# retrojetpacks/Gadget-Leicester

Measured on AMD Instinct MI355X. Metric: particle-steps/sec (gravity+SPH), higher is better.
Workload: dtype f64

## Files before the change

gadget-leicester_amd/csrc/ghip_walk.h:

```cpp
#pragma once
#include "ghip_internal.h"
#include "ghip_count.h"

#ifndef GHIP_WALK_WAVES
#define GHIP_WALK_WAVES 8
#endif
#ifndef GHIP_WALK_OPT
#define GHIP_WALK_OPT 15
#endif


struct GravK
{
  double theta;
  double errtol;
  double boxsize, boxhalf;
  int periodic, unequal;
  int debug_steps;
  int xcd_remap;
  double rcut, rcut2, asmthfac;
  double fac_intp;
  double k1875;
};

__device__ int *d_walk_errw = nullptr;

#include "ghip_walkrec.h"

typedef double v16i __attribute__((ext_vector_type(8)));

struct __attribute__((aligned(8))) EwPair
{
  double lo, hi;
};
__device__ __forceinline__ EwPair d_ldpair(const double *p)
{
  return *reinterpret_cast<const EwPair *>(p);
}

__device__ __forceinline__ double d_f64(const v16i &v, int i)
{
  return v[i];
}
__device__ __forceinline__ int d_lo32(const v16i &v, int i)
{
  return __double2loint(v[i]);
}
__device__ __forceinline__ int d_hi32(const v16i &v, int i)
{
  return __double2hiint(v[i]);
}

__device__ __forceinline__ unsigned int d_rec_off(int e)
{
  return (unsigned int) __builtin_amdgcn_readfirstlane(e) << 6;
}
template <class T>
__device__ __forceinline__ void d_load1(const T *__restrict__ base, int e, v16i &R)
{
  const unsigned int off = d_rec_off(e);
  asm volatile("s_load_dwordx16 %0, %1, %2\n\ts_waitcnt lgkmcnt(0)" : "=s"(R) : "s"(base), "s"(off) : "memory");
}
template <class T>
__device__ __forceinline__ void d_load2(const T *__restrict__ base, int ea, v16i &A, int eb, v16i &B)
{
  const unsigned int oa = d_rec_off(ea), ob = d_rec_off(eb);
  asm volatile("s_load_dwordx16 %0, %2, %3\n\ts_load_dwordx16 %1, %2, %4\n\ts_waitcnt lgkmcnt(0)"
               : "=&s"(A), "=&s"(B)
               : "s"(base), "s"(oa), "s"(ob)
               : "memory");
}
template <class T>
__device__ __forceinline__ void d_touch_next(const T *__restrict__ base, unsigned int off, int &scratch)
{
  asm volatile("s_load_dword %0, %1, %2 offset:0x40" : "=s"(scratch) : "s"(base), "s"(off) : "memory");
}
template <class T>
__device__ __forceinline__ void d_touch(const T *__restrict__ base, int e, int &scratch)
{
  const unsigned int off = d_rec_off(e);
  asm volatile("s_load_dword %0, %1, %2" : "=s"(scratch) : "s"(base), "s"(off) : "memory");
}
template <class T>
__device__ __forceinline__ void d_load1_touch(const T *__restrict__ base, unsigned int off, v16i &R,
                                              int &s1, int &s2)
{
  asm volatile("s_load_dwordx16 %0, %3, %4\n\ts_waitcnt lgkmcnt(0)"
               : "=s"(R), "+s"(s1), "+s"(s2)
               : "s"(base), "s"(off)
               : "memory");
}
__device__ __forceinline__ void d_drain_touch(int &s1, int &s2)
{
  asm volatile("s_waitcnt lgkmcnt(0) ; drain-touches" : "+s"(s1), "+s"(s2) : : "memory");
}

__device__ __forceinline__ double d_rsqrt(double x)
{
  double y = __builtin_amdgcn_rsq(x);
  double t = x * y;
  double e = fma(-t, y, 1.0);
  double p = fma(0.375, e, 0.5);
  return fma(y * e, p, y);
}

__device__ __forceinline__ double d_mass_over_r3(double mass, double x, double k15 = 1.5,
                                                 double k1875 = 1.875)
{
  double y = __builtin_amdgcn_rsq(x);
  double y2 = y * y;
  double e = fma(-x, y2, 1.0);
  double p = fma(k1875, e, k15);
  double c = (mass * y) * y2;
  return fma(c * e, p, c);
}

__device__ __forceinline__ double d_grav_fac(double mass, double r2, double h, double h2,
                                             double &r_out)
{
  if(r2 >= h2)
    {
      double rinv = d_rsqrt(r2);
      r_out = r2 * rinv;
      return mass * rinv * rinv * rinv;
    }
  double r = sqrt(r2);
  r_out = r;
  double h_inv = 1.0 / h;
  double h3_inv = h_inv * h_inv * h_inv;
  double u = r * h_inv;
  if(u < 0.5)
    return mass * h3_inv * (10.666666666667 + u * u * (32.0 * u - 38.4));
  return mass * h3_inv *
         (21.333333333333 - 48.0 * u + 38.4 * u * u - 10.666666666667 * u * u * u -
          0.066666666667 / (u * u * u));
}

template <bool BRICK>
__device__ __forceinline__ void d_ewald_interp(const double *__restrict__ tab, double fac_intp,
                                               double dx, double dy, double dz, double &fx,
                                               double &fy, double &fz)
{
  const int E1 = GHIP_EN + 1;
  const double sx = dx < 0 ? 1.0 : -1.0, sy = dy < 0 ? 1.0 : -1.0, sz = dz < 0 ? 1.0 : -1.0;
  dx = fabs(dx);
  dy = fabs(dy);
  dz = fabs(dz);
  double u = dx * fac_intp;
  int i = (int) u;
  if(i >= GHIP_EN)
    i = GHIP_EN - 1;
  u -= i;
  double v = dy * fac_intp;
  int j = (int) v;
  if(j >= GHIP_EN)
    j = GHIP_EN - 1;
  v -= j;
  double w = dz * fac_intp;
  int k = (int) w;
  if(k >= GHIP_EN)
    k = GHIP_EN - 1;
  w -= k;
  double f1 = (1 - u) * (1 - v) * (1 - w), f2 = (1 - u) * (1 - v) * (w);
  double f3 = (1 - u) * (v) * (1 - w), f4 = (1 - u) * (v) * (w);
  double f5 = (u) * (1 - v) * (1 - w), f6 = (u) * (1 - v) * (w);
  double f7 = (u) * (v) * (1 - w), f8 = (u) * (v) * (w);
  EwPair x00, x01, x10, x11, y00, y01, y10, y11, z00, z01, z10, z11;
  if(!BRICK)
    {
      const unsigned int ui = (unsigned int) i, uj = (unsigned int) j, uk = (unsigned int) k;
      const unsigned int R1 = E1 * 8u, R2 = E1 * E1 * 8u;
      const unsigned int ox = (ui * E1 + uj) * R1 + uk * 8u;
      const unsigned int oy = (uj * E1 + ui) * R1 + uk * 8u;
      const unsigned int oz = (uk * E1 + uj) * R1 + ui * 8u;
      const unsigned int ox2 = ox + R2, oy2 = oy + R2, oz2 = oz + R2;
      const char *tb = reinterpret_cast<const char *>(tab);
#define EW_LD(off, imm) d_ldpair(reinterpret_cast<const double *>(tb + (size_t) (off) + (imm)))
      x00 = EW_LD(ox, 0), x01 = EW_LD(ox, R1), x10 = EW_LD(ox2, 0), x11 = EW_LD(ox2, R1);
      y00 = EW_LD(oy, 0), y01 = EW_LD(oy, R1), y10 = EW_LD(oy2, 0), y11 = EW_LD(oy2, R1);
      z00 = EW_LD(oz, 0), z01 = EW_LD(oz, R1), z10 = EW_LD(oz2, 0), z11 = EW_LD(oz2, R1);
#undef EW_LD
    }
  else
    {
      const unsigned int SA = GHIP_EW_NB * GHIP_EW_NKB * 128, SB = GHIP_EW_NKB * 128;
      const unsigned int ai = (i >> 1) * SA + (i & 1) * 64, ai1 = ((i + 1) >> 1) * SA + ((i + 1) & 1) * 64;
      const unsigned int aj = (j >> 1) * SA + (j & 1) * 64, aj1 = ((j + 1) >> 1) * SA + ((j + 1) & 1) * 64;
      const unsigned int ak = (k >> 1) * SA + (k & 1) * 64, ak1 = ((k + 1) >> 1) * SA + ((k + 1) & 1) * 64;
      const unsigned int bi = (i >> 1) * SB + (i & 1) * 32, bi1 = ((i + 1) >> 1) * SB + ((i + 1) & 1) * 32;
      const unsigned int bj = (j >> 1) * SB + (j & 1) * 32, bj1 = ((j + 1) >> 1) * SB + ((j + 1) & 1) * 32;
      const unsigned int ck = ((((unsigned int) k * 43u) >> 7) * 13u + (unsigned int) k) * 8u;
      const unsigned int ci = ((((unsigned int) i * 43u) >> 7) * 13u + (unsigned int) i) * 8u;
      const char *tb = reinterpret_cast<const char *>(tab);
#define EW_LD(off) d_ldpair(reinterpret_cast<const double *>(tb + (off)))
      x00 = EW_LD(ai + bj + ck), x01 = EW_LD(ai + bj1 + ck), x10 = EW_LD(ai1 + bj + ck),
      x11 = EW_LD(ai1 + bj1 + ck);
      y00 = EW_LD(aj + bi + ck), y01 = EW_LD(aj + bi1 + ck), y10 = EW_LD(aj1 + bi + ck),
      y11 = EW_LD(aj1 + bi1 + ck);
      z00 = EW_LD(ak + bj + ci), z01 = EW_LD(ak + bj1 + ci), z10 = EW_LD(ak1 + bj + ci),
      z11 = EW_LD(ak1 + bj1 + ci);
#undef EW_LD
    }
  fx = sx * (x00.lo * f1 + x00.hi * f2 + x01.lo * f3 + x01.hi * f4 + x10.lo * f5 + x10.hi * f6 +
             x11.lo * f7 + x11.hi * f8);
  fy = sy * (y00.lo * f1 + y00.hi * f2 + y10.lo * f3 + y10.hi * f4 + y01.lo * f5 + y01.hi * f6 +
             y11.lo * f7 + y11.hi * f8);
  fz = sz * (z00.lo * f1 + z10.lo * f2 + z01.lo * f3 + z11.lo * f4 + z00.hi * f5 + z10.hi * f6 +
             z01.hi * f7 + z11.hi * f8);
}

struct WalkLane
{
  double pos_x, pos_y, pos_z, h_i, aold;
  double h2;
  double k15;
  double acc_x, acc_y, acc_z;
  int nint;
};

__device__ __forceinline__ double d_nearest1(double x, double boxsize, double boxhalf)
{
  return (fabs(x) > boxhalf) ? x - copysign(boxsize, x) : x;
}

__device__ __forceinline__ double d_nearest1_masked(double x, double boxsize, double boxhalf)
{
  if(fabs(x) > boxhalf)
    {
      x -= copysign(boxsize, x);
      asm volatile("" : "+v"(x));
    }
  return x;
}

typedef unsigned long long lmask;
#define D_BAL(cond) __builtin_amdgcn_ballot_w64(cond)
#define D_LANE(mask) __builtin_amdgcn_inverse_ballot_w64(mask)

__device__ __forceinline__ void d_skip_to(int &my_skip, int skip)
{
  asm volatile("v_max_i32 %0, %1, %0" : "+v"(my_skip) : "s"(skip));
}

template <int MODE, bool PERIODIC, bool UNEQUAL, bool OWNED, bool REL>
__device__ __forceinline__ int d_walk_element(int e, const v16i &H,
                                              const WalkCold *__restrict__ cold, const GravK &p,
                                              const float *__restrict__ srtab,
                                              const double *__restrict__ ewtab, WalkLane &W,
                                              int &my_skip)
{
  const double ex = d_f64(H, 0), ey = d_f64(H, 1), ez = d_f64(H, 2), mass = d_f64(H, 3);
  const double mlen2 = d_f64(H, 4), len2 = d_f64(H, 5);
  const int skip = d_lo32(H, 6), pidx = d_hi32(H, 6);
  const double aux = d_f64(H, 7);
  const lmask act = D_BAL(e >= my_skip);
  int next;

  double dx = ex - W.pos_x, dy = ey - W.pos_y, dz = ez - W.pos_z;
  double r2;
  if((GHIP_WALK_OPT & 1) && (MODE == GHIP_WALK_EWALD || PERIODIC))
    {
      r2 = dx * dx + dy * dy + dz * dz;
      if(D_BAL(r2 >= p.boxhalf * p.boxhalf) != 0)
        {
          if(D_LANE(D_BAL(fabs(dx) > p.boxhalf)))
            {
              dx -= copysign(p.boxsize, dx);
              asm volatile("" : "+v"(dx));
            }
          if(D_LANE(D_BAL(fabs(dy) > p.boxhalf)))
            {
              dy -= copysign(p.boxsize, dy);
              asm volatile("" : "+v"(dy));
            }
          if(D_LANE(D_BAL(fabs(dz) > p.boxhalf)))
            {
              dz -= copysign(p.boxsize, dz);
              asm volatile("" : "+v"(dz));
            }
          r2 = dx * dx + dy * dy + dz * dz;
        }
    }
  else if(MODE == GHIP_WALK_EWALD || PERIODIC)
    {
      const lmask wx = D_BAL(fabs(dx) > p.boxhalf), wy = D_BAL(fabs(dy) > p.boxhalf),
                  wz = D_BAL(fabs(dz) > p.boxhalf);
      if((wx | wy | wz) != 0)
        {
          if(D_LANE(wx))
            {
              dx -= copysign(p.boxsize, dx);
              asm volatile("" : "+v"(dx));
            }
          if(D_LANE(wy))
            {
              dy -= copysign(p.boxsize, dy);
              asm volatile("" : "+v"(dy));
            }
          if(D_LANE(wz))
            {
              dz -= copysign(p.boxsize, dz);
              asm volatile("" : "+v"(dz));
            }
        }
      r2 = dx * dx + dy * dy + dz * dz;
    }
  else
    r2 = dx * dx + dy * dy + dz * dz;
  double h = W.h_i, h2 = W.h2;
  lmask interact;

  if(pidx >= 0)
    {
      next = e + 1;
      interact = act;
      if(MODE != GHIP_WALK_EWALD && UNEQUAL)
        {
          if(h < aux)
            {
              h = aux;
              h2 = h * h;
            }
        }
    }
  else
    {
      lmask gt, rel;
      if(REL)
        {
          gt = D_BAL(mlen2 > r2 * r2 * W.aold);
          rel = ~0ull;
        }
      else
        {
          gt = D_BAL(len2 > r2 * p.theta * p.theta);
          rel = 0ull;
        }
      lmask open = act & gt;
      lmask far = act & ~gt & rel;
      lmask drop = 0;
      const double len2x4 = __hiloint2double(d_hi32(H, 5) + 0x00200000, d_lo32(H, 5));
      const lmask boxcand = far & D_BAL(r2 < len2x4);
      lmask cutcand = 0;
      if(MODE == GHIP_WALK_SHORTRANGE)
        cutcand = act & D_BAL(r2 > p.rcut2);
      lmask need_cold = boxcand;
      if(MODE == GHIP_WALK_SHORTRANGE)
        need_cold |= cutcand;
      if(MODE == GHIP_WALK_EWALD)
        need_cold |= open;
      if(need_cold != 0)
        {
          v16i C;
          d_load1(cold, e, C);
          const double cx = d_f64(C, 0), cy = d_f64(C, 1), cz = d_f64(C, 2), len = d_f64(C, 3);
          const double len06 = d_f64(C, 4);
          const double c0 = cx - W.pos_x, c1 = cy - W.pos_y, c2 = cz - W.pos_z;
          if(MODE == GHIP_WALK_SHORTRANGE)
            {
              if(cutcand != 0)
                {
                  double eff = p.rcut + 0.5 * len;
                  double d0 = c0, d1 = c1, d2 = c2;
                  if(PERIODIC)
                    {
                      d0 = d_nearest1(d0, p.boxsize, p.boxhalf);
                      d1 = d_nearest1(d1, p.boxsize, p.boxhalf);
                      d2 = d_nearest1(d2, p.boxsize, p.boxhalf);
                    }
                  drop = cutcand &
                         (D_BAL(fabs(d0) > eff) | D_BAL(fabs(d1) > eff) | D_BAL(fabs(d2) > eff));
                }
              open &= ~drop;
              far &= ~drop;
            }
          if(far != 0)
            open |= far & D_BAL(fabs(c0) < len06) & D_BAL(fabs(c1) < len06) &
                    D_BAL(fabs(c2) < len06);
          if(MODE == GHIP_WALK_EWALD)
            {
              if(open != 0 && !(len > 0.20 * p.boxsize))
                {
                  double u0 = d_nearest1(c0, p.boxsize, p.boxhalf);
                  double u1 = d_nearest1(c1, p.boxsize, p.boxhalf);
                  double u2 = d_nearest1(c2, p.boxsize, p.boxhalf);
                  double lim = 0.5 * (p.boxsize - len);
                  open &= D_BAL(fabs(u0) > lim) | D_BAL(fabs(u1) > lim) | D_BAL(fabs(u2) > lim);
                }
            }
        }
      if(MODE != GHIP_WALK_EWALD && UNEQUAL)
        {
          const double ms = fabs(aux);
          const lmask up = act & ~drop & ~open & D_BAL(h < ms);
          if(up != 0)
            {
              if(D_LANE(up))
                {
                  h = ms;
                  h2 = ms * ms;
                }
              if(aux < 0)
                open |= up & D_BAL(r2 < ms * ms);
            }
        }
      interact = act & ~drop & ~open;
      if(!((GHIP_WALK_OPT & 4) && OWNED && MODE == GHIP_WALK_NEWTON) || (interact & D_BAL(r2 < h2)) != 0)
        if(D_LANE(interact | drop))
          d_skip_to(my_skip, skip);
      next = skip;
      if(open != 0)
        {
          next = e + 1;
          if(skip == next)
            {
              int *w = *(int *volatile *) &d_walk_errw;
              if(w)
                *(volatile int *) w = 1;
            }
        }
    }

  if(OWNED && MODE == GHIP_WALK_NEWTON && (interact & D_BAL(r2 < h2)) == 0)
    {
      const int counted = pidx & 1;
      const int sk = skip;
      if(D_LANE(interact))
        {
          const double fac = (GHIP_WALK_OPT & 8) ? d_mass_over_r3(mass, r2, W.k15, p.k1875)
                                                 : d_mass_over_r3(mass, r2);
          W.acc_x += dx * fac;
          W.acc_y += dy * fac;
          W.acc_z += dz * fac;
          if(GHIP_WALK_OPT & 2)
            W.nint += counted;
          else
            W.nint += (mass > 0) ? 1 : 0;
          if(GHIP_WALK_OPT & 4)
            d_skip_to(my_skip, sk);
        }
      return next;
    }
  if(OWNED && D_LANE(interact))
    {
      if(MODE == GHIP_WALK_EWALD)
        {
          double fx, fy, fz;
          d_ewald_interp<UNEQUAL>(ewtab, p.fac_intp, dx, dy, dz, fx, fy, fz);
          W.acc_x += mass * fx;
          W.acc_y += mass * fy;
          W.acc_z += mass * fz;
          W.nint++;
        }
      else
        {
          double r;
          double fac = d_grav_fac(mass, r2, h, h2, r);
          if(MODE == GHIP_WALK_SHORTRANGE)
            {
              int tabindex = (int) (p.asmthfac * r);
              if(tabindex < GHIP_NTAB)
                {
                  fac *= srtab[tabindex];
                  W.acc_x += dx * fac;
                  W.acc_y += dy * fac;
                  W.acc_z += dz * fac;
                  W.nint++;
                }
            }
          else
            {
              W.acc_x += dx * fac;
              W.acc_y += dy * fac;
              W.acc_z += dz * fac;
              if(mass > 0)
                W.nint++;
            }
        }
    }
  return next;
}

struct WalkPlan
{
  int nwaves;
  const int *__restrict__ wave_bucket;
  const int *__restrict__ woff;
  const int *__restrict__ nsub;
  unsigned int *__restrict__ steps_out;
  unsigned int *started;
  int started_at;
};

struct SegCursor
{
  int kseg;
  int e, s1;
};

template <int MODE, bool PERIODIC, bool UNEQUAL, bool REL>
__device__ __forceinline__ bool d_enter_segment(SegCursor &c, int stride, const WalkSeg &sg,
                                                const WalkHot *__restrict__ hot,
                                                const WalkCold *__restrict__ cold, const GravK &p,
                                                const float *__restrict__ srtab,
                                                const double *__restrict__ ewtab, bool valid,
                                                WalkLane &W, int &my_skip, unsigned int &steps)
{
  while(c.kseg < sg.ns)
    {
      const int s0 = __builtin_amdgcn_readfirstlane(sg.start[c.kseg]);
      c.s1 = __builtin_amdgcn_readfirstlane(sg.start[c.kseg + 1]);
      my_skip = valid ? 0 : 0x7fffffff;
      const int na = __builtin_amdgcn_readfirstlane(sg.nanc[c.kseg]);
      for(int a = 0; a < na; a++)
        {
          int ea = __builtin_amdgcn_readfirstlane(sg.anc[c.kseg * GHIP_MAXANC + a]);
          v16i H;
          d_load1(hot, ea, H);
          d_walk_element<MODE, PERIODIC, UNEQUAL, false, REL>(ea, H, cold, p, srtab, ewtab, W, my_skip);
          steps++;
        }
      int first = d_wave_min_i32(my_skip);
      c.e = __builtin_amdgcn_readfirstlane(first > s0 ? first : s0);
      if(c.e < c.s1)
        return true;
      c.kseg += stride;
    }
  return false;
}

template <int MODE, bool PERIODIC, bool UNEQUAL, bool REL>
__device__ __forceinline__ void d_walk_run(const WalkSeg &sg, int sub, const WalkHot *__restrict__ hot,
                                           const WalkCold *__restrict__ cold, const GravK &p,
                                           const float *__restrict__ srtab,
                                           const double *__restrict__ ewtab, bool valid, WalkLane &W,
                                           unsigned int &steps)
{
  if(MODE != GHIP_WALK_EWALD)
    {
      SegCursor A;
      int skipA = 0;
      A.kseg = sub;
      const int stride = sg.nsub;
      bool liveA = d_enter_segment<MODE, PERIODIC, UNEQUAL, REL>(A, stride, sg, hot, cold, p, srtab,
                                                            ewtab, valid, W, skipA, steps);
      int t1 = 0, t2 = 0;
      while(liveA)
        {
          v16i HA;
          const unsigned int offA = d_rec_off(A.e);
          d_load1_touch(hot, offA, HA, t1, t2);
          d_touch_next(hot, offA, t1);
          d_touch(hot, d_lo32(HA, 6), t2);
          steps++;
          A.e = __builtin_amdgcn_readfirstlane(
            d_walk_element<MODE, PERIODIC, UNEQUAL, true, REL>(A.e, HA, cold, p, srtab, ewtab, W, skipA));
          if(A.e >= A.s1)
            {
              d_drain_touch(t1, t2);
              A.kseg += stride;
              liveA = d_enter_segment<MODE, PERIODIC, UNEQUAL, REL>(A, stride, sg, hot, cold, p, srtab,
                                                               ewtab, valid, W, skipA, steps);
            }
        }
      d_drain_touch(t1, t2);
    }
  else
    {
      SegCursor A, B;
      int skipA = 0, skipB = 0;
      A.kseg = sub;
      B.kseg = sub + sg.nsub;
      const int stride = 2 * sg.nsub;
      bool liveA = d_enter_segment<MODE, PERIODIC, UNEQUAL, REL>(A, stride, sg, hot, cold, p, srtab, ewtab, valid,
                                                   W, skipA, steps);
      bool liveB = d_enter_segment<MODE, PERIODIC, UNEQUAL, REL>(B, stride, sg, hot, cold, p, srtab, ewtab, valid,
                                                   W, skipB, steps);
      while(liveA && liveB)
        {
          v16i HA, HB;
          d_load2(hot, A.e, HA, B.e, HB);
          steps += 2;
          A.e = __builtin_amdgcn_readfirstlane(
            d_walk_element<MODE, PERIODIC, UNEQUAL, true, REL>(A.e, HA, cold, p, srtab, ewtab, W, skipA));
          B.e = __builtin_amdgcn_readfirstlane(
            d_walk_element<MODE, PERIODIC, UNEQUAL, true, REL>(B.e, HB, cold, p, srtab, ewtab, W, skipB));
          if(A.e >= A.s1)
            {
              A.kseg += stride;
              liveA = d_enter_segment<MODE, PERIODIC, UNEQUAL, REL>(A, stride, sg, hot, cold, p, srtab, ewtab,
                                                      valid, W, skipA, steps);
            }
          if(B.e >= B.s1)
            {
              B.kseg += stride;
              liveB = d_enter_segment<MODE, PERIODIC, UNEQUAL, REL>(B, stride, sg, hot, cold, p, srtab, ewtab,
                                                      valid, W, skipB, steps);
            }
        }
      if(liveB)
        {
          A = B;
          skipA = skipB;
          liveA = true;
        }
      while(liveA)
        {
          v16i HA;
          d_load1(hot, A.e, HA);
          steps++;
          A.e = __builtin_amdgcn_readfirstlane(
            d_walk_element<MODE, PERIODIC, UNEQUAL, true, REL>(A.e, HA, cold, p, srtab, ewtab, W, skipA));
          if(A.e >= A.s1)
            {
              A.kseg += stride;
              liveA = d_enter_segment<MODE, PERIODIC, UNEQUAL, REL>(A, stride, sg, hot, cold, p, srtab, ewtab,
                                                      valid, W, skipA, steps);
            }
        }
    }

}

template <int MODE, bool PERIODIC, bool UNEQUAL>
__global__ void __launch_bounds__(GHIP_BLOCK) __attribute__((amdgpu_waves_per_eu(MODE == GHIP_WALK_EWALD ? 4 : GHIP_WALK_WAVES, 8)))
k_grav_walk(int nelem, const WalkHot *__restrict__ hot, const WalkCold *__restrict__ cold,
            WalkSeg sg, int nt, const int *__restrict__ tgt, const double *__restrict__ tx,
            const double *__restrict__ ty, const double *__restrict__ tz,
            const double *__restrict__ tsoft, const double *__restrict__ toldacc, GravK p,
            const float *__restrict__ srtab, const double *__restrict__ ewtab,
            double *__restrict__ pax, double *__restrict__ pay, double *__restrict__ paz,
            int *__restrict__ pcost, unsigned long long *__restrict__ counter,
            unsigned long long *__restrict__ acc, WalkPlan plan)
{
  const int lane = threadIdx.x & 63;
  if(plan.started && blockIdx.x == plan.started_at && threadIdx.x == 0)
    __hip_atomic_store(plan.started, 1u, __ATOMIC_RELEASE, __HIP_MEMORY_SCOPE_SYSTEM);
  const int per_xcd = gridDim.x >> 3;
  int lblock = blockIdx.x;
  if(p.xcd_remap == 1)
    lblock = (blockIdx.x & 7) * per_xcd + (blockIdx.x >> 3);
  else if(p.xcd_remap > 1)
    {
      const int j = blockIdx.x >> 3, x = blockIdx.x & 7, G = p.xcd_remap;
      lblock = ((j / G) * 8 + x) * G + (j % G);
    }
  const int wave = __builtin_amdgcn_readfirstlane((lblock * (int) blockDim.x + threadIdx.x) >> 6);
  if(wave >= plan.nwaves)
    return;
  const int bucket = __builtin_amdgcn_readfirstlane(plan.wave_bucket[wave]);
  if(bucket < 0 || bucket * 64 >= nt)
    return;
  const int sub = wave - __builtin_amdgcn_readfirstlane(plan.woff[bucket]);
  sg.nsub = __builtin_amdgcn_readfirstlane(plan.nsub[bucket]);
  const int ti = bucket * 64 + lane;
  const bool valid = ti < nt;
  const int s = valid ? (tgt ? tgt[ti] : ti) : 0;

  WalkLane W;
  W.pos_x = W.pos_y = W.pos_z = 0;
  W.h_i = 1;
  W.aold = 0;
  W.h2 = 1;
  if(valid)
    {
      W.pos_x = tx[s];
      W.pos_y = ty[s];
      W.pos_z = tz[s];
      W.h_i = tsoft[s];
      W.aold = p.errtol * toldacc[s];
      W.h2 = W.h_i * W.h_i;
    }
  W.acc_x = W.acc_y = W.acc_z = 0;
  W.nint = 0;
  W.k15 = 1.5;
  asm volatile("" : "+v"(W.k15));
  unsigned int steps = 0;

  if(p.theta == 0)
    d_walk_run<MODE, PERIODIC, UNEQUAL, true>(sg, sub, hot, cold, p, srtab, ewtab, valid, W, steps);
  else
    d_walk_run<MODE, PERIODIC, UNEQUAL, false>(sg, sub, hot, cold, p, srtab, ewtab, valid, W, steps);

  if(valid)
    {
      const size_t o = (size_t) wave * 64 + lane;
      pax[o] = W.acc_x;
      pay[o] = W.acc_y;
      paz[o] = W.acc_z;
      pcost[o] = p.debug_steps ? (int) steps : W.nint;
    }
  unsigned long long tot = d_wave_sum_u64((unsigned long long) W.nint);
  if(lane == 0 && tot && counter)
    {
      d_count(counter, 0, tot);
      d_count(acc, 0, tot);
    }
  if(lane == 0)
    {
      if(counter)
        {
          d_count(counter, 1, (unsigned long long) steps);
          d_count(acc, 1, (unsigned long long) steps);
        }
      atomicAdd(plan.steps_out + bucket, steps);
    }
}

__global__ void k_plan_nsub(int nb, int ns, int sbase, const unsigned int *__restrict__ steps_prev,
                            int nprev, int *__restrict__ nsub)
{
  __shared__ unsigned long long part[4];
  unsigned long long tot = 0;
  if(nprev > 0)
    {
      for(int k = threadIdx.x; k < nprev; k += blockDim.x)
        tot += steps_prev[k];
      for(int o = 32; o > 0; o >>= 1)
        tot += __shfl_xor(tot, o);
      if((threadIdx.x & 63) == 0)
        part[threadIdx.x >> 6] = tot;
      __syncthreads();
      tot = part[0] + part[1] + part[2] + part[3];
    }
  int b = blockIdx.x * blockDim.x + threadIdx.x;
  if(b >= nb)
    return;
  int s = ns < sbase ? ns : sbase;
  if(b < nprev && tot > 0)
    {
      double mean = (double) tot / (double) nprev;
      s = (int) ((double) sbase * (double) steps_prev[b] / mean) + 1;
      s = s < 2 ? 2 : s;
      s = s > 64 ? 64 : s;
      if(s > ns)
        s = ns;
    }
  nsub[b] = s < 1 ? 1 : s;
}

__global__ void k_plan_fill(int nb, const int *__restrict__ nsub, const int *__restrict__ woff,
                            int maxwaves, int *__restrict__ wave_bucket,
                            unsigned int *__restrict__ steps_out, int *__restrict__ errword)
{
  int b = blockIdx.x * blockDim.x + threadIdx.x;
  if(b >= nb)
    return;
  int o = woff[b], s = nsub[b];
  if(o + s > maxwaves)
    *(volatile int *) errword = 1;
  for(int q = 0; q < s; q++)
    if(o + q < maxwaves)
      wave_bucket[o + q] = b;
  steps_out[b] = 0;
}

struct SegTables
{
  int ntab;
  int ns[3], soff[3], noff[3];
};

__global__ void k_build_segments(const TreeSizes *__restrict__ ts, const int4 *__restrict__ lk,
                                 SegTables T, int *__restrict__ start, int *__restrict__ nanc,
                                 int *__restrict__ anc)
{
  const int nelem = ts->nelem;
  int g = blockIdx.x * blockDim.x + threadIdx.x;
  int j = 0;
  while(j < T.ntab && g > T.ns[j])
    {
      g -= T.ns[j] + 1;
      j++;
    }
  if(j >= T.ntab)
    return;
  const int ns = T.ns[j], k = g;
  start += T.soff[j];
  nanc += T.noff[j];
  anc += (size_t) T.noff[j] * GHIP_MAXANC;
  long long chunk = ((long long) nelem + ns - 1) / ns;
  long long s0l = (long long) k * chunk;
  int s0 = (int) (s0l > nelem ? nelem : s0l);
  if(k == ns)
    s0 = nelem;
  start[k] = s0;
  if(k == ns)
    return;
  int na = 0, e = 0;
  while(e < s0)
    {
      int4 q = lk[e];
      if(!LK_IS_PARTICLE(q) && q.x > s0)
        {
          if(na < GHIP_MAXANC)
            anc[k * GHIP_MAXANC + na] = e;
          na++;
          e = e + 1;
        }
      else
        e = q.x;
    }
  nanc[k] = na < GHIP_MAXANC ? na : GHIP_MAXANC;
}

__global__ void k_combine_grav(int nt, WalkPlan plan, const int *__restrict__ tgt,
                               const int *__restrict__ perm, const double *__restrict__ pax,
                               const double *__restrict__ pay, const double *__restrict__ paz,
                               const int *__restrict__ pcost, int n, double *__restrict__ oacc,
                               int *__restrict__ ocost, int accumulate, int debug_max)
{
  int ti = blockIdx.x * blockDim.x + threadIdx.x;
  if(ti >= nt)
    return;
  const int bucket = ti >> 6, lane = ti & 63;
  const int w0 = plan.woff[bucket];
  int nsub = plan.nsub[bucket];
  if(w0 + nsub > plan.nwaves)
    nsub = plan.nwaves > w0 ? plan.nwaves - w0 : 0;
  double a0 = 0, a1 = 0, a2 = 0;
  int c = 0;
  for(int s = 0; s < nsub; s++)
    {
      size_t o = (size_t) (w0 + s) * 64 + lane;
      a0 += pax[o];
      a1 += pay[o];
      a2 += paz[o];
      c = debug_max ? (pcost[o] > c ? pcost[o] : c) : c + pcost[o];
    }
  int i = perm ? perm[tgt[ti]] : ti;
  if(accumulate)
    {
      oacc[i] += a0;
      oacc[(size_t) n + i] += a1;
      oacc[2 * (size_t) n + i] += a2;
      ocost[i] += c;
    }
  else
    {
      oacc[i] = a0;
      oacc[(size_t) n + i] = a1;
      oacc[2 * (size_t) n + i] = a2;
      ocost[i] = c;
    }
}

__global__ void k_combine_pair(int nt, WalkPlan pn, WalkPlan pe, const int *__restrict__ tgt,
                               const int *__restrict__ perm, const double *__restrict__ nax,
                               const double *__restrict__ nay, const double *__restrict__ naz,
                               const int *__restrict__ ncost, const double *__restrict__ eax,
                               const double *__restrict__ eay, const double *__restrict__ eaz,
                               const int *__restrict__ ecost, int n, double *__restrict__ oacc,
                               int *__restrict__ ocost)
{
  int ti = blockIdx.x * blockDim.x + threadIdx.x;
  if(ti >= nt)
    return;
  const int bucket = ti >> 6, lane = ti & 63;
  double a0 = 0, a1 = 0, a2 = 0, b0 = 0, b1 = 0, b2 = 0;
  int c = 0, d = 0;
  {
    const int w0 = pn.woff[bucket];
    int nsub = pn.nsub[bucket];
    if(w0 + nsub > pn.nwaves)
      nsub = pn.nwaves > w0 ? pn.nwaves - w0 : 0;
    for(int s = 0; s < nsub; s++)
      {
        size_t o = (size_t) (w0 + s) * 64 + lane;
        a0 += nax[o];
        a1 += nay[o];
        a2 += naz[o];
        c += ncost[o];
      }
  }
  {
    const int w0 = pe.woff[bucket];
    int nsub = pe.nsub[bucket];
    if(w0 + nsub > pe.nwaves)
      nsub = pe.nwaves > w0 ? pe.nwaves - w0 : 0;
    for(int s = 0; s < nsub; s++)
      {
        size_t o = (size_t) (w0 + s) * 64 + lane;
        b0 += eax[o];
        b1 += eay[o];
        b2 += eaz[o];
        d += ecost[o];
      }
  }
  int i = perm ? perm[tgt[ti]] : ti;
  oacc[i] = a0 + b0;
  oacc[(size_t) n + i] = a1 + b1;
  oacc[2 * (size_t) n + i] = a2 + b2;
  ocost[i] = c + d;
}

__global__ void k_fill_elems(const TreeSizes *__restrict__ ts, const double4 *__restrict__ xm,
                             const double4 *__restrict__ cl, const int4 *__restrict__ lk,
                             const double *__restrict__ aux, WalkHot *__restrict__ hot,
                             WalkCold *__restrict__ cold)
{
  int e = blockIdx.x * blockDim.x + threadIdx.x;
  if(e >= ts->nelem)
    return;
  double4 v = xm[e], c = cl[e];
  int4 k = lk[e];
  WalkHot h;
  h.x = v.x;
  h.y = v.y;
  h.z = v.z;
  h.m = v.w;
  WalkCold q;
  q.cx = c.x;
  q.cy = c.y;
  q.cz = c.z;
  q.len = c.w;
  if(LK_IS_PARTICLE(k))
    {
      h.mlen2 = 0.0;
      h.len2 = 0.0;
      q.len06 = 0.0;
    }
  else
    {
      h.mlen2 = v.w * c.w * c.w;
      h.len2 = c.w * c.w;
      q.len06 = 0.60 * c.w;
    }
  h.skip = k.x;
  h.pidx = (LK_IS_PARTICLE(k) ? 0 : (int) 0x80000000) | (v.w > 0 ? 1 : 0);
  h.aux = aux[e];
  q.spare[0] = q.spare[1] = q.spare[2] = 0.0;
  hot[e] = h;
  cold[e] = q;
}
```

Baseline: 83.12 million.

## Restructure Ewald table addressing and move skip updates into interaction blocks

Moves the Ewald table address computation into a shared helper that uses 24-bit multiplies and a base offset plus immediate form, so the 12 loads can use constant offsets. In the tree walk, the per-lane skip-pointer update is moved into the force-accumulation branches for Newton and Ewald modes. The softened Newton case gets its own branch instead of falling through to the general path. It also switches to a masked nearest-image helper in the Ewald opening test. The goal is fewer address instructions and less divergent control flow per walk step. The cost is extra branches, and the result relies on the new helpers producing the same addresses as before.

```diff
diff --git a/gadget-leicester_amd/csrc/ghip_ewaddr.h b/gadget-leicester_amd/csrc/ghip_ewaddr.h
--- /dev/null
+++ b/gadget-leicester_amd/csrc/ghip_ewaddr.h
@@ -0,0 +1,54 @@
+#pragma once
+
+#if defined(__HIP_DEVICE_COMPILE__) && __HIP_DEVICE_COMPILE__
+#define GHIP_EW_UMUL(a, b) __umul24((a), (b))
+#define GHIP_EW_IMUL(a, b) __mul24((a), (b))
+#else
+#define GHIP_EW_UMUL(a, b) ((unsigned int) (a) * (unsigned int) (b))
+#define GHIP_EW_IMUL(a, b) ((int) (a) * (int) (b))
+#endif
+#ifdef __HIPCC__
+#define GHIP_EW_FN static inline __host__ __device__ __attribute__((always_inline))
+#else
+#define GHIP_EW_FN static inline
+#endif
+
+GHIP_EW_FN void ghip_ew_brick_addr(int i, int j, int k, unsigned int off[12], unsigned int imm[12])
+{
+  const unsigned int SA = GHIP_EW_NB * GHIP_EW_NKB * 128, SB = GHIP_EW_NKB * 128;
+  const unsigned int ui = (unsigned int) i, uj = (unsigned int) j, uk = (unsigned int) k;
+  const int pi = i & 1, pj = j & 1, pk = k & 1;
+  const unsigned int ai = (unsigned int) (GHIP_EW_IMUL(pi, 64 - (int) (SA / 2)) + (int) GHIP_EW_UMUL(ui, SA / 2));
+  const unsigned int aj = (unsigned int) (GHIP_EW_IMUL(pj, 64 - (int) (SA / 2)) + (int) GHIP_EW_UMUL(uj, SA / 2));
+  const unsigned int ak = (unsigned int) (GHIP_EW_IMUL(pk, 64 - (int) (SA / 2)) + (int) GHIP_EW_UMUL(uk, SA / 2));
+  const unsigned int ai1 = GHIP_EW_UMUL((unsigned int) pi, SA - 128) + ai;
+  const unsigned int aj1 = GHIP_EW_UMUL((unsigned int) pj, SA - 128) + aj;
+  const unsigned int ak1 = GHIP_EW_UMUL((unsigned int) pk, SA - 128) + ak;
+  const unsigned int bi = (unsigned int) (GHIP_EW_IMUL(pi, 32 - (int) (SB / 2)) + (int) GHIP_EW_UMUL(ui, SB / 2));
+  const unsigned int bj = (unsigned int) (GHIP_EW_IMUL(pj, 32 - (int) (SB / 2)) + (int) GHIP_EW_UMUL(uj, SB / 2));
+  const unsigned int bi1 = GHIP_EW_UMUL((unsigned int) pi, SB - 64) + bi;
+  const unsigned int bj1 = GHIP_EW_UMUL((unsigned int) pj, SB - 64) + bj;
+  const unsigned int ck = (GHIP_EW_UMUL(GHIP_EW_UMUL(uk, 43u) >> 7, 13u) + uk) * 8u;
+  const unsigned int ci = (GHIP_EW_UMUL(GHIP_EW_UMUL(ui, 43u) >> 7, 13u) + ui) * 8u;
+  off[0] = ai + bj + ck, off[1] = ai + bj1 + ck, off[2] = ai1 + bj + ck, off[3] = ai1 + bj1 + ck;
+  off[4] = aj + bi + ck, off[5] = aj + bi1 + ck, off[6] = aj1 + bi + ck, off[7] = aj1 + bi1 + ck;
+  off[8] = ak + bj + ci, off[9] = ak + bj1 + ci, off[10] = ak1 + bj + ci, off[11] = ak1 + bj1 + ci;
+  for(int q = 0; q < 12; q++)
+    imm[q] = (q & 1) * 32u + ((q >> 1) & 1) * 64u;
+}
+
+GHIP_EW_FN void ghip_ew_rows_addr(int i, int j, int k, unsigned int off[12], unsigned int imm[12])
+{
+  const unsigned int R1 = (GHIP_EN + 1) * 8u, R2 = (GHIP_EN + 1) * (GHIP_EN + 1) * 8u;
+  const unsigned int ui = (unsigned int) i, uj = (unsigned int) j, uk = (unsigned int) k;
+  const unsigned int E1 = GHIP_EN + 1;
+  const unsigned int ox = GHIP_EW_UMUL(GHIP_EW_UMUL(ui, E1) + uj, R1) + uk * 8u;
+  const unsigned int oy = GHIP_EW_UMUL(GHIP_EW_UMUL(uj, E1) + ui, R1) + uk * 8u;
+  const unsigned int oz = GHIP_EW_UMUL(GHIP_EW_UMUL(uk, E1) + uj, R1) + ui * 8u;
+  for(int q = 0; q < 12; q++)
+    {
+      const unsigned int o = q < 4 ? ox : q < 8 ? oy : oz;
+      off[q] = o + ((q >> 1) & 1) * R2;
+      imm[q] = (q & 1) * R1;
+    }
+}
diff --git a/gadget-leicester_amd/csrc/ghip_walk.h b/gadget-leicester_amd/csrc/ghip_walk.h
--- a/gadget-leicester_amd/csrc/ghip_walk.h
+++ b/gadget-leicester_amd/csrc/ghip_walk.h
@@ -1,6 +1,7 @@
 #pragma once
 #include "ghip_internal.h"
 #include "ghip_count.h"
+#include "ghip_ewaddr.h"
 
 #ifndef GHIP_WALK_WAVES
 #define GHIP_WALK_WAVES 8
@@ -166,41 +167,17 @@
   double f5 = (u) * (1 - v) * (1 - w), f6 = (u) * (1 - v) * (w);
   double f7 = (u) * (v) * (1 - w), f8 = (u) * (v) * (w);
   EwPair x00, x01, x10, x11, y00, y01, y10, y11, z00, z01, z10, z11;
-  if(!BRICK)
-    {
-      const unsigned int ui = (unsigned int) i, uj = (unsigned int) j, uk = (unsigned int) k;
-      const unsigned int R1 = E1 * 8u, R2 = E1 * E1 * 8u;
-      const unsigned int ox = (ui * E1 + uj) * R1 + uk * 8u;
-      const unsigned int oy = (uj * E1 + ui) * R1 + uk * 8u;
-      const unsigned int oz = (uk * E1 + uj) * R1 + ui * 8u;
-      const unsigned int ox2 = ox + R2, oy2 = oy + R2, oz2 = oz + R2;
-      const char *tb = reinterpret_cast<const char *>(tab);
-#define EW_LD(off, imm) d_ldpair(reinterpret_cast<const double *>(tb + (size_t) (off) + (imm)))
-      x00 = EW_LD(ox, 0), x01 = EW_LD(ox, R1), x10 = EW_LD(ox2, 0), x11 = EW_LD(ox2, R1);
-      y00 = EW_LD(oy, 0), y01 = EW_LD(oy, R1), y10 = EW_LD(oy2, 0), y11 = EW_LD(oy2, R1);
-      z00 = EW_LD(oz, 0), z01 = EW_LD(oz, R1), z10 = EW_LD(oz2, 0), z11 = EW_LD(oz2, R1);
+  unsigned int off[12], imm[12];
+  if(BRICK)
+    ghip_ew_brick_addr(i, j, k, off, imm);
+  else
+    ghip_ew_rows_addr(i, j, k, off, imm);
+  const char *tb = reinterpret_cast<const char *>(tab);
+#define EW_LD(q) d_ldpair(reinterpret_cast<const double *>(tb + (size_t) off[q] + imm[q]))
+  x00 = EW_LD(0), x01 = EW_LD(1), x10 = EW_LD(2), x11 = EW_LD(3);
+  y00 = EW_LD(4), y01 = EW_LD(5), y10 = EW_LD(6), y11 = EW_LD(7);
+  z00 = EW_LD(8), z01 = EW_LD(9), z10 = EW_LD(10), z11 = EW_LD(11);
 #undef EW_LD
-    }
-  else
-    {
-      const unsigned int SA = GHIP_EW_NB * GHIP_EW_NKB * 128, SB = GHIP_EW_NKB * 128;
-      const unsigned int ai = (i >> 1) * SA + (i & 1) * 64, ai1 = ((i + 1) >> 1) * SA + ((i + 1) & 1) * 64;
-      const unsigned int aj = (j >> 1) * SA + (j & 1) * 64, aj1 = ((j + 1) >> 1) * SA + ((j + 1) & 1) * 64;
-      const unsigned int ak = (k >> 1) * SA + (k & 1) * 64, ak1 = ((k + 1) >> 1) * SA + ((k + 1) & 1) * 64;
-      const unsigned int bi = (i >> 1) * SB + (i & 1) * 32, bi1 = ((i + 1) >> 1) * SB + ((i + 1) & 1) * 32;
-      const unsigned int bj = (j >> 1) * SB + (j & 1) * 32, bj1 = ((j + 1) >> 1) * SB + ((j + 1) & 1) * 32;
-      const unsigned int ck = ((((unsigned int) k * 43u) >> 7) * 13u + (unsigned int) k) * 8u;
-      const unsigned int ci = ((((unsigned int) i * 43u) >> 7) * 13u + (unsigned int) i) * 8u;
-      const char *tb = reinterpret_cast<const char *>(tab);
-#define EW_LD(off) d_ldpair(reinterpret_cast<const double *>(tb + (off)))
-      x00 = EW_LD(ai + bj + ck), x01 = EW_LD(ai + bj1 + ck), x10 = EW_LD(ai1 + bj + ck),
-      x11 = EW_LD(ai1 + bj1 + ck);
-      y00 = EW_LD(aj + bi + ck), y01 = EW_LD(aj + bi1 + ck), y10 = EW_LD(aj1 + bi + ck),
-      y11 = EW_LD(aj1 + bi1 + ck);
-      z00 = EW_LD(ak + bj + ci), z01 = EW_LD(ak + bj1 + ci), z10 = EW_LD(ak1 + bj + ci),
-      z11 = EW_LD(ak1 + bj1 + ci);
-#undef EW_LD
-    }
   fx = sx * (x00.lo * f1 + x00.hi * f2 + x01.lo * f3 + x01.hi * f4 + x10.lo * f5 + x10.hi * f6 +
              x11.lo * f7 + x11.hi * f8);
   fy = sy * (y00.lo * f1 + y00.hi * f2 + y10.lo * f3 + y10.hi * f4 + y01.lo * f5 + y01.hi * f6 +
@@ -309,6 +286,7 @@
     r2 = dx * dx + dy * dy + dz * dz;
   double h = W.h_i, h2 = W.h2;
   lmask interact;
+  lmask took = 0;
 
   if(pidx >= 0)
     {
@@ -381,9 +359,9 @@
             {
               if(open != 0 && !(len > 0.20 * p.boxsize))
                 {
-                  double u0 = d_nearest1(c0, p.boxsize, p.boxhalf);
-                  double u1 = d_nearest1(c1, p.boxsize, p.boxhalf);
-                  double u2 = d_nearest1(c2, p.boxsize, p.boxhalf);
+                  double u0 = d_nearest1_masked(c0, p.boxsize, p.boxhalf);
+                  double u1 = d_nearest1_masked(c1, p.boxsize, p.boxhalf);
+                  double u2 = d_nearest1_masked(c2, p.boxsize, p.boxhalf);
                   double lim = 0.5 * (p.boxsize - len);
                   open &= D_BAL(fabs(u0) > lim) | D_BAL(fabs(u1) > lim) | D_BAL(fabs(u2) > lim);
                 }
@@ -405,9 +383,7 @@
             }
         }
       interact = act & ~drop & ~open;
-      if(!((GHIP_WALK_OPT & 4) && OWNED && MODE == GHIP_WALK_NEWTON) || (interact & D_BAL(r2 < h2)) != 0)
-        if(D_LANE(interact | drop))
-          d_skip_to(my_skip, skip);
+      took = interact | drop;
       next = skip;
       if(open != 0)
         {
@@ -421,11 +397,34 @@
         }
     }
 
-  if(OWNED && MODE == GHIP_WALK_NEWTON && (interact & D_BAL(r2 < h2)) == 0)
-    {
+  const bool skip_in_block =
+    OWNED && ((MODE == GHIP_WALK_NEWTON && (GHIP_WALK_OPT & 4)) || MODE == GHIP_WALK_EWALD);
+  if(!skip_in_block)
+    if(D_LANE(took))
+      d_skip_to(my_skip, skip);
+
+  if(OWNED && MODE == GHIP_WALK_NEWTON)
+    {
+      lmask plain = interact;
+      if((interact & D_BAL(r2 < h2)) != 0)
+        {
+          if(D_LANE(interact))
+            {
+              double r;
+              const double fac = d_grav_fac(mass, r2, h, h2, r);
+              W.acc_x += dx * fac;
+              W.acc_y += dy * fac;
+              W.acc_z += dz * fac;
+              if(mass > 0)
+                W.nint++;
+              if(GHIP_WALK_OPT & 4)
+                d_skip_to(my_skip, skip);
+            }
+          plain = 0;
+        }
       const int counted = pidx & 1;
       const int sk = skip;
-      if(D_LANE(interact))
+      if(D_LANE(plain))
         {
           const double fac = (GHIP_WALK_OPT & 8) ? d_mass_over_r3(mass, r2, W.k15, p.k1875)
                                                  : d_mass_over_r3(mass, r2);
@@ -451,6 +450,7 @@
           W.acc_y += mass * fy;
           W.acc_z += mass * fz;
           W.nint++;
+          d_skip_to(my_skip, skip);
         }
       else
         {
```

Result: no change. 82.38 million (-0.9%).
